# nuggy875/NeRF_pytorch_paeng

Hardware: AMD Instinct MI355X
Metric: rays/sec (4096-ray batch, 64c+128f samples) + 800×800 frame render ms (higher is better)
Workload: dtype f32

## Files before the change

nerf_pytorch_paeng_amd/csrc/layout.h:

```cpp
#pragma once
#include <stdint.h>
#include <stddef.h>

namespace minerf {

constexpr int QUAD_BYTES = 1024;
constexpr int SLOT_QUADS = 16;
constexpr int SLOT_BYTES = QUAD_BYTES * SLOT_QUADS;
constexpr int HEADER_BYTES = 1024;
constexpr uint32_t BLOB_MAGIC = 0x4D494E46u;

__host__ __device__ constexpr int pe_ksteps(int L) { return ((3 * L + 2 + 3) / 4) * 4; }

constexpr int KERNEL_LX = 10, KERNEL_LD = 4;

constexpr int MAX_KERNEL_WIDTH = 512;
__host__ __device__ constexpr int kernel_width(int W) { return W <= 128 ? 128 : (W <= 256 ? 256 : (W <= 384 ? 384 : 512)); }
__host__ __device__ constexpr bool wide_kernel_width(int Wk) { return Wk > 256; }
__host__ __device__ constexpr int pe_ksteps16(int L) { return (((3 * L + 1) / 2 + 1 + 3) / 4) * 4; }
__host__ __device__ constexpr bool native_width(int W) { return W == 128 || W == 256; }

struct BlobLayout {
    uint32_t stream_off;
    uint32_t stream_bytes_hoist;
    uint32_t stream_bytes_full;
    uint32_t side_off;
    uint32_t side_floats;
    uint32_t bias_trunk;
    uint32_t bias_feat;
    uint32_t bias_d;
    uint32_t dens_w;
    uint32_t dens_b;
    uint32_t color_w;
    uint32_t color_b;
    uint32_t wdir_t;
    uint32_t total_bytes;
};

__host__ __device__ inline uint32_t round_up_u32(uint32_t v, uint32_t m) { return (v + m - 1) / m * m; }

inline BlobLayout make_layout(int D, int W_net, int skip, int , int ) {
    constexpr int L_x = KERNEL_LX, L_d = KERNEL_LD;
    const int W = kernel_width(W_net);
    BlobLayout b{};
    const int NT = W / 32;
    const int in_d = 3 + 6 * L_d;
    const uint32_t pe_quads = (uint32_t)(pe_ksteps(L_x) / 4) * NT;
    const uint32_t h_quads = (uint32_t)(W / 2 / 4) * NT;
    uint32_t quads = pe_quads;
    for (int l = 1; l < D; ++l) quads += h_quads + ((skip >= 0 && l == skip + 1) ? pe_quads : 0);
    quads += h_quads;
    quads += (uint32_t)(W / 2 / 4) * (NT / 2);
    b.stream_off = HEADER_BYTES;
    b.stream_bytes_hoist = round_up_u32(quads, SLOT_QUADS) * QUAD_BYTES;
    uint32_t full = round_up_u32(quads, SLOT_QUADS) + round_up_u32((uint32_t)(pe_ksteps(L_d) / 4) * (NT / 2), SLOT_QUADS);
    b.stream_bytes_full = full * QUAD_BYTES;
    b.side_off = b.stream_off + b.stream_bytes_full;
    uint32_t f = 0;
    b.bias_trunk = f; f += (uint32_t)D * W;
    b.bias_feat = f;  f += W;
    b.bias_d = f;     f += W / 2;
    b.dens_w = f;     f += W;
    b.dens_b = f;     f += 4;
    b.color_w = f;    f += 3 * (W / 2);
    b.color_b = f;    f += 4;
    b.wdir_t = f;     f += (uint32_t)in_d * (W / 2);
    b.side_floats = round_up_u32(f, 4);
    b.total_bytes = b.side_off + b.side_floats * 4;
    return b;
}

struct ParamOffsets {
    uint32_t w_x[16], b_x[16];
    int in_l[16];
    uint32_t w_d, b_d, w_feat, b_feat, w_dens, b_dens, w_color, b_color;
    uint32_t total;
};

inline ParamOffsets make_param_offsets(int D, int W, int skip, int L_x, int L_d) {
    ParamOffsets p{};
    const int in_x = 3 + 6 * L_x, in_d = 3 + 6 * L_d;
    uint32_t f = 0;
    for (int l = 0; l < D; ++l) {
        p.in_l[l] = (l == 0) ? in_x : ((skip >= 0 && l == skip + 1) ? W + in_x : W);
        p.w_x[l] = f; f += (uint32_t)W * p.in_l[l];
        p.b_x[l] = f; f += W;
    }
    p.w_d = f;     f += (uint32_t)(W / 2) * (W + in_d);
    p.b_d = f;     f += W / 2;
    p.w_feat = f;  f += (uint32_t)W * W;
    p.b_feat = f;  f += W;
    p.w_dens = f;  f += W;
    p.b_dens = f;  f += 1;
    p.w_color = f; f += 3 * (W / 2);
    p.b_color = f; f += 3;
    p.total = f;
    return p;
}

inline uint32_t bwd_stream_bytes(int D, int W) {
    const uint32_t NT = W / 32;
    const uint32_t quads = (uint32_t)(W / 16) * NT + (uint32_t)D * (uint32_t)(W / 8) * NT;
    return round_up_u32(quads, SLOT_QUADS) * QUAD_BYTES;
}
// ... 3 lines not shown
```

nerf_pytorch_paeng_amd/csrc/mlp_train.hip:

```cpp
#include <type_traits>
#include <vector>
#include "mlp_core.h"

namespace minerf {

int stage_embed(const float*, const float*, int64_t, int, int, int, float*, hipStream_t);
int dgrad_f16s(const mi_nerf_net*, const void*, const float*, const float*, const float*, const unsigned*, const unsigned*, float*, float*, float*, int64_t, int,
               long long, long long, const unsigned*, hipStream_t);

struct DgradArgs {
    const char* stream;
    unsigned stream_bytes;
    const float* side;
    unsigned side_floats, o_dens_w, o_color_w;
    const float* d_raw;
    const unsigned* mask_h;
    const unsigned* mask_g;
    float* delta_h;
    float* delta_f;
    float* delta_d;
    long long P;
    long long n_valid;
    long long n_wtiles;
    int S, tpr;
// ... 66 lines not shown
                    h2[4 * q + e] = mask_apply(v, q, e, mg);
                }
            }
        }
        acc_zero<NT>(acc);
        {
            float* row = a.delta_d + idx * (W / 2) + 4 * hh;
            auto hook = [&](int kq, int t) __attribute__((always_inline)) { if (t == NT - 1) store_chunk(h2, kq, row); };
            gemm_part<NT, HN / 2, NT, AL>(acc, h2, aq, smem, ring, lane, hook);
        }
        acc_to_b<NT, false>(acc, h);
        acc_zero<NT>(acc);
        {
            float* row = a.delta_f + idx * W + 4 * hh;
            auto hook = [&](int kq, int t) __attribute__((always_inline)) { if (t == NT - 1) store_chunk(h, kq, row); };
            gemm_part<NT, HN, NT, AL>(acc, h, aq, smem, ring, lane, hook);
        }
        {
            const unsigned mw[4] = {mhv[0], mhv[1], mhv[2], mhv[3]};
            if (a.D > 1) mhv = *(const u32x4*)(a.mask_h + (((long long)(a.D - 2) * a.n_wtiles + wt) * 64 + lane) * 4);
            const float ds = dr[3];
#pragma unroll
            for (int q = 0; q < 4 * NT; ++q) {
                const f32x4 wv = *(const f32x4*)(dw + 8 * q + 4 * hh);
#pragma unroll
                for (int e = 0; e < 4; ++e)
                    h[4 * q + e] = mask_apply(__builtin_fmaf(wv[e], ds, acc[q >> 2][4 * (q & 3) + e]), q, e, mw);
            }
        }
#pragma unroll 1
        for (int l = a.D - 1; l > 0; --l) {
            float* row = a.delta_h + ((long long)l * a.P + idx) * W + 4 * hh;
            acc_zero<NT>(acc);
            auto hook = [&](int kq, int t) __attribute__((always_inline)) { if (t == NT - 1) store_chunk(h, kq, row); };
            gemm_part<NT, HN, NT, AL>(acc, h, aq, smem, ring, lane, hook);
            const unsigned mw[4] = {mhv[0], mhv[1], mhv[2], mhv[3]};
            if (l > 1) mhv = *(const u32x4*)(a.mask_h + (((long long)(l - 2) * a.n_wtiles + wt) * 64 + lane) * 4);
#pragma unroll
            for (int q = 0; q < 4 * NT; ++q)
#pragma unroll
                for (int e = 0; e < 4; ++e) h[4 * q + e] = mask_apply(acc[q >> 2][4 * (q & 3) + e], q, e, mw);
        }
        store_rows<NT>(h, a.delta_h + idx * W + 4 * hh, valid);
    }
    asm volatile("s_waitcnt vmcnt(0)" ::: "memory");
    __syncthreads();
}

constexpr int WG_MAXB = 12;
struct WgradArgs {
    const float* dlt[WG_MAXB]; const float* x[WG_MAXB];
    int ldd[WG_MAXB], ldx[WG_MAXB], M[WG_MAXB], N[WG_MAXB];
    int want_bias[WG_MAXB];
    long long P;
    float* partial;
    float* bpartial;
    int slices;
};
struct ReduceBatch {
    float* out[WG_MAXB]; float* bias[WG_MAXB];
    int ldo[WG_MAXB], M[WG_MAXB], N[WG_MAXB];
};

typedef unsigned u32x4 __attribute__((ext_vector_type(4)));
__device__ __forceinline__ __amdgpu_buffer_rsrc_t wg_rsrc(const float* base, long long row0, long long ld, long long P, int rows) {
    long long left = P - row0;
    left = left < 0 ? 0 : (left > rows ? rows : left);
    return __builtin_amdgcn_make_buffer_rsrc((void*)(base + row0 * ld), 0, (int)(left * ld * 4), 0x00020000);
}
__global__ __launch_bounds__(256) __attribute__((amdgpu_waves_per_eu(1, 1)))
void wgrad_big_kernel(const WgradArgs a) {
    constexpr int U = 6;
    __shared__ f32x4 bshare[2][64];
    const int lane = threadIdx.x & 63;
    const int wave = __builtin_amdgcn_readfirstlane(threadIdx.x >> 6);
    const int i = lane & 31, kh = lane >> 5;
    const unsigned nwg = gridDim.x * gridDim.y, v = blockIdx.y * gridDim.x + blockIdx.x;
    const unsigned xcd = v & 7, slot = v >> 3;
    const unsigned full = nwg >> 3, rem = nwg & 7;
    const unsigned flat = xcd * full + (xcd < rem ? xcd : rem) + slot;
    const int b = (int)(flat / gridDim.x);
    const unsigned slice = flat - (unsigned)b * gridDim.x;
    const int wm = wave >> 1, wn = wave & 1;
    const int m0 = wm * 128, n0 = wn * 128;
    const bool aok = m0 + 4 * i < a.M[b], bok = n0 + 4 * i < a.N[b];
    const float* abase = a.dlt[b];
    const float* bbase = a.x[b];
    const long long ldd = a.ldd[b], ldx = a.ldx[b];
    const bool want_bias = a.want_bias[b] != 0;

    f32x16 acc[4][4];
#pragma unroll
    for (int tm = 0; tm < 4; ++tm)
#pragma unroll
        for (int tn = 0; tn < 4; ++tn)
#pragma unroll
            for (int r = 0; r < 16; ++r) acc[tm][tn][r] = 0.0f;
    f32x4 bsum = {0.f, 0.f, 0.f, 0.f};

    const long long slices = gridDim.x;
    unsigned voa[U], vob[U];
#pragma unroll
    for (int u = 0; u < U; ++u) {
        voa[u] = aok ? (unsigned)(((2 * u + kh) * ldd + m0 + 4 * i) * 4) : 0x80000000u;
        vob[u] = bok ? (unsigned)(((2 * u + kh) * ldx + n0 + 4 * i) * 4) : 0x80000000u;
    }
    long long req_group = slice;
    f32x4 ca[U], cb[U], na[U], nb[U], fa[U], fb[U];
    __amdgpu_buffer_rsrc_t ra, rb;
    auto open_group = [&]() __attribute__((always_inline)) {
        const long long row0 = req_group * (2 * U);
        ra = wg_rsrc(abase, row0, ldd, a.P, 2 * U);
        rb = wg_rsrc(bbase, row0, ldx, a.P, 2 * U);
        req_group += slices;
    };
    auto request = [&](int u, f32x4& A, f32x4& B) __attribute__((always_inline)) {
        A = __builtin_bit_cast(f32x4, __builtin_amdgcn_raw_buffer_load_b128(ra, voa[u], 0, 0));
        B = __builtin_bit_cast(f32x4, __builtin_amdgcn_raw_buffer_load_b128(rb, vob[u], 0, 0));
    };
    open_group();
#pragma unroll
    for (int u = 0; u < U; ++u) request(u, ca[u], cb[u]);
    open_group();
#pragma unroll
    for (int u = 0; u < U; ++u) request(u, na[u], nb[u]);
    auto step = [&](auto PAR, f32x4 (&A)[U], f32x4 (&B)[U], f32x4 (&FA)[U], f32x4 (&FB)[U]) __attribute__((always_inline)) {
        constexpr int par = decltype(PAR)::value;
        open_group();
#pragma unroll
        for (int u = 0; u < U; ++u) {
#pragma unroll
            for (int tm = 0; tm < 4; ++tm)
#pragma unroll
                for (int tn = 0; tn < 4; ++tn)
                    acc[tm][tn] = __builtin_amdgcn_mfma_f32_32x32x2f32(A[u][tm], B[u][tn], acc[tm][tn], 0, 0, 0);
            if ((u & 1) == par) bsum += A[u];
            request(u, FA[u], FB[u]);
            __builtin_amdgcn_sched_barrier(0);
        }
    };
    const long long all_groups = (a.P + 2 * U - 1) / (2 * U);
    const long long n_groups = (all_groups + slices - 1) / slices;
    auto loop = [&](auto PAR) __attribute__((always_inline)) {
        long long g = 0;
        do {
            step(PAR, ca, cb, fa, fb);
            step(PAR, na, nb, ca, cb);
            step(PAR, fa, fb, na, nb);
            g += 3;
        } while (g < n_groups);
    };
    if (!want_bias) loop(std::integral_constant<int, -1>{});
    else if (wn == 0) loop(std::integral_constant<int, 0>{});
    else loop(std::integral_constant<int, 1>{});
    const int lane_o = (int)__builtin_amdgcn_mbcnt_hi(~0u, __builtin_amdgcn_mbcnt_lo(~0u, 0u));
    const int i_o = lane_o & 31, kh_o = lane_o >> 5;
    float* out = a.partial + ((size_t)b * a.slices + slice) * (256 * 256);
// ... 8 lines not shown
            *(f32x4*)(out + (size_t)m * 256 + n0 + 4 * i_o) = v;
        }
    if (want_bias) {
        if (wn == 1) bshare[wm][lane_o] = bsum;
        __syncthreads();
        if (wn == 0) {
            bsum += bshare[wm][lane_o];
            f32x4 sv;
#pragma unroll
            for (int e = 0; e < 4; ++e) sv[e] = bsum[e] + __shfl_xor(bsum[e], 32, 64);
            if (kh_o == 0) *(f32x4*)(a.bpartial + ((size_t)b * a.slices + slice) * 256 + m0 + 4 * i_o) = sv;
        }
    }
}

typedef _Float16 f16x8 __attribute__((ext_vector_type(8)));
__global__ __launch_bounds__(256) void absmax_kernel(const float* __restrict__ x, long long n, unsigned* __restrict__ out_bits) {
    float m = 0.0f;
    const long long n4 = ((uintptr_t)x & 15) == 0 ? n >> 2 : 0;
    for (long long i = (long long)blockIdx.x * 256 + threadIdx.x; i < n4; i += (long long)gridDim.x * 256) {
        const f32x4 v = ((const f32x4*)x)[i];
        m = __builtin_fmaxf(__builtin_fmaxf(m, __builtin_fmaxf(__builtin_fabsf(v[0]), __builtin_fabsf(v[1]))), __builtin_fmaxf(__builtin_fabsf(v[2]), __builtin_fabsf(v[3])));
    }
    for (long long i = 4 * n4 + (long long)blockIdx.x * 256 + threadIdx.x; i < n; i += (long long)gridDim.x * 256) m = __builtin_fmaxf(m, __builtin_fabsf(x[i]));
#pragma unroll
    for (int o = 32; o > 0; o >>= 1) m = __builtin_fmaxf(m, __shfl_xor(m, o, 64));
    if ((threadIdx.x & 63) == 0 && m == m) atomicMax(out_bits, __float_as_uint(m));
}
static void launch_absmax(const float* x, long long n, unsigned* out_bits, hipStream_t st) {
    long long blocks = (n / 4 + 255) / 256;
    blocks = blocks < 1 ? 1 : (blocks > 4096 ? 4096 : blocks);
    hipLaunchKernelGGL(absmax_kernel, dim3((unsigned)blocks), dim3(256), 0, st, x, n, out_bits);
}
template <bool S>
__device__ __forceinline__ void split_pair(float v0, float v1, float s, unsigned& hi, unsigned& lo) {
    if constexpr (S) { v0 *= s; v1 *= s; }
    asm("v_cvt_pk_f16_f32 %0, %1, %2" : "=v"(hi) : "v"(v0), "v"(v1));
    asm("v_fma_mixlo_f16 %0, %1, -1.0, %2 op_sel_hi:[1,0,0]\n\tv_fma_mixhi_f16 %0, %1, -1.0, %3 op_sel:[1,0,0] op_sel_hi:[1,0,0]"
        : "=&v"(lo) : "v"(hi), "v"(v0), "v"(v1));
}
template <int BIAS>
__device__ __forceinline__ void wgrad_f16s_body(const WgradArgs& a, const unsigned* absmax_bits, f32x4 (*bshare)[64]) {
    const int lane = threadIdx.x & 63;
    const int wave = __builtin_amdgcn_readfirstlane(threadIdx.x >> 6);
    const int i = lane & 31, kh = lane >> 5;
    const unsigned nwg = gridDim.x * gridDim.y, v = blockIdx.y * gridDim.x + blockIdx.x;
    const unsigned xcd = v & 7, slot = v >> 3;
    const unsigned full = nwg >> 3, rem = nwg & 7;
    const unsigned flat = xcd * full + (xcd < rem ? xcd : rem) + slot;
    const int b = (int)(flat / gridDim.x);
    const unsigned slice = flat - (unsigned)b * gridDim.x;
    const int wm = wave >> 1, wn = wave & 1;
    const int m0 = wm * 128, n0 = wn * 128;
    const bool aok = m0 + 4 * i < a.M[b], bok = n0 + 4 * i < a.N[b];
    const float* abase = a.dlt[b];
    const float* bbase = a.x[b];
    const long long ldd = a.ldd[b], ldx = a.ldx[b];
    const unsigned mb = __builtin_amdgcn_readfirstlane((int)*absmax_bits);
    int e = (int)((mb >> 23) & 255u) - 127;
    if (mb == 0u || e < -100) e = -100;
    if (e > 100) e = 100;
    const float sc = __uint_as_float((unsigned)(127 + 7 - e) << 23), inv_sc = __uint_as_float((unsigned)(127 - 7 + e) << 23);

    f32x16 acc[4][4];
#pragma unroll
    for (int tm = 0; tm < 4; ++tm)
#pragma unroll
        for (int tn = 0; tn < 4; ++tn)
#pragma unroll
            for (int r = 0; r < 16; ++r) acc[tm][tn][r] = 0.0f;
    f32x4 bsum = {0.f, 0.f, 0.f, 0.f};

    constexpr int GROUP = 32;
    const long long slices = gridDim.x;
    unsigned voa[4], vob[4];
#pragma unroll
    for (int r = 0; r < 4; ++r) {
        voa[r] = aok ? (unsigned)(((8 * kh + r) * ldd + m0 + 4 * i) * 4) : 0x80000000u;
        vob[r] = bok ? (unsigned)(((8 * kh + r) * ldx + n0 + 4 * i) * 4) : 0x80000000u;
    }
    long long req_group = slice;
    struct Unit { f32x4 A[4], B[4]; };
    auto request = [&](int q, Unit& u) __attribute__((always_inline)) {
        const long long row0 = req_group * GROUP + 16 * (q >> 1) + 4 * (q & 1);
        const __amdgpu_buffer_rsrc_t ra = wg_rsrc(abase, row0, ldd, a.P, 12), rb = wg_rsrc(bbase, row0, ldx, a.P, 12);
#pragma unroll
        for (int r = 0; r < 4; ++r) {
            u.A[r] = __builtin_bit_cast(f32x4, __builtin_amdgcn_raw_buffer_load_b128(ra, voa[r], 0, 0));
            u.B[r] = __builtin_bit_cast(f32x4, __builtin_amdgcn_raw_buffer_load_b128(rb, vob[r], 0, 0));
        }
    };
    auto open_group = [&]() __attribute__((always_inline)) { req_group += slices; };
    unsigned ahi[4][4], alo[4][4], bhi[4][4], blo[4][4];
    auto convert = [&](int h, const Unit& u) __attribute__((always_inline)) {
#pragma unroll
        for (int t = 0; t < 4; ++t)
#pragma unroll
            for (int pr = 0; pr < 2; ++pr) {
                split_pair<true>(u.A[2 * pr][t], u.A[2 * pr + 1][t], sc, ahi[t][2 * h + pr], alo[t][2 * h + pr]);
                split_pair<false>(u.B[2 * pr][t], u.B[2 * pr + 1][t], 1.0f, bhi[t][2 * h + pr], blo[t][2 * h + pr]);
            }
        if constexpr (BIAS) {
#pragma unroll
            for (int r = 0; r < 4; ++r) bsum += u.A[r];
        }
    };
    auto mfmas = [&]() __attribute__((always_inline)) {
        f16x8 AH[4], AL[4], BH[4], BL[4];
#pragma unroll
        for (int t = 0; t < 4; ++t) {
            u32x4 w;
            w[0] = ahi[t][0]; w[1] = ahi[t][1]; w[2] = ahi[t][2]; w[3] = ahi[t][3]; AH[t] = __builtin_bit_cast(f16x8, w);
            w[0] = alo[t][0]; w[1] = alo[t][1]; w[2] = alo[t][2]; w[3] = alo[t][3]; AL[t] = __builtin_bit_cast(f16x8, w);
            w[0] = bhi[t][0]; w[1] = bhi[t][1]; w[2] = bhi[t][2]; w[3] = bhi[t][3]; BH[t] = __builtin_bit_cast(f16x8, w);
            w[0] = blo[t][0]; w[1] = blo[t][1]; w[2] = blo[t][2]; w[3] = blo[t][3]; BL[t] = __builtin_bit_cast(f16x8, w);
        }
#pragma unroll
        for (int tm = 0; tm < 4; ++tm)
#pragma unroll
            for (int tn = 0; tn < 4; ++tn) {
                acc[tm][tn] = __builtin_amdgcn_mfma_f32_32x32x16_f16(AH[tm], BH[tn], acc[tm][tn], 0, 0, 0);
                acc[tm][tn] = __builtin_amdgcn_mfma_f32_32x32x16_f16(AH[tm], BL[tn], acc[tm][tn], 0, 0, 0);
                acc[tm][tn] = __builtin_amdgcn_mfma_f32_32x32x16_f16(AL[tm], BH[tn], acc[tm][tn], 0, 0, 0);
            }
    };
    Unit u0, u1, u2, u3;
    request(0, u0); request(1, u1); request(2, u2); request(3, u3);
    const long long all_groups = (a.P + GROUP - 1) / GROUP;
    const long long n_groups = (all_groups + slices - 1) / slices;
    for (long long g = 0; g < n_groups; ++g) {
        open_group();
// ... 165 lines not shown
#pragma unroll
    for (int q = 0; q < NN; ++q) {
        const float v = nsum[q] + __shfl_xor(nsum[q], 32, 64);
        if (kh == 0) sums[wave * (Wp + Np) + Wp + 32 * q + i] = v;
    }
    __syncthreads();
    for (int c = threadIdx.x; c < Wp + Np; c += 256) {
        const float v = ((sums[c] + sums[(Wp + Np) + c]) + sums[2 * (Wp + Np) + c]) + sums[3 * (Wp + Np) + c];
        if (c < Wp) { if (a.wsum) a.wsum[(size_t)blockIdx.x * Wp + c] = v; }
        else if (a.nsum) a.nsum[(size_t)blockIdx.x * Np + (c - Wp)] = v;
    }
}

__global__ __launch_bounds__(256) void reduce_partial_kernel(const float* __restrict__ partial, const float* __restrict__ bpartial,
                                                              int slices, int Mp, int Np, int M, int N, float* __restrict__ out, int ldo,
                                                              float* __restrict__ bias, int bias_pitch, int transposed) {
    __shared__ float red[4][64];
    const int g = threadIdx.x >> 6, o = threadIdx.x & 63;
    const int idx = blockIdx.x * 64 + o;
    const int total = M * N + (bias ? M : 0);
    float acc = 0.0f;
    if (idx < M * N) {
        const int m = idx / N, n = idx - m * N;
        const float* p = partial + (transposed ? (size_t)n * Np + m : (size_t)m * Np + n);
        const size_t stride = (size_t)Mp * Np;
        float s[8] = {0.f, 0.f, 0.f, 0.f, 0.f, 0.f, 0.f, 0.f};
        int sl = g;
        for (; sl + 28 < slices; sl += 32) {
#pragma unroll
            for (int k = 0; k < 8; ++k) s[k] += p[(size_t)(sl + 4 * k) * stride];
        }
        for (; sl < slices; sl += 4) s[0] += p[(size_t)sl * stride];
        acc = ((s[0] + s[1]) + (s[2] + s[3])) + ((s[4] + s[5]) + (s[6] + s[7]));
    } else if (idx < total) {
        const int m = idx - M * N;
        for (int sl = g; sl < slices; sl += 4) acc += bpartial[(size_t)sl * bias_pitch + m];
    }
    red[g][o] = acc;
    __syncthreads();
    if (g == 0 && idx < total) {
        const float v = ((red[0][o] + red[1][o]) + red[2][o]) + red[3][o];
        if (idx < M * N) { const int m = idx / N, n = idx - m * N; out[(size_t)m * ldo + n] = v; }
        else bias[idx - M * N] = v;
    }
}

__global__ __launch_bounds__(256) void reduce_batch_kernel(const float* __restrict__ partial, const float* __restrict__ bpartial, int slices,
                                                            const ReduceBatch rb) {
    __shared__ float red[4][64];
    const int b = blockIdx.y;
    const int M = rb.M[b], N = rb.N[b];
    const int g = threadIdx.x >> 6, o = threadIdx.x & 63;
    const int idx = blockIdx.x * 64 + o;
    const int total = M * N + (rb.bias[b] ? M : 0);
    float acc = 0.0f;
    if (idx < M * N) {
        const int m = idx / N, n = idx - m * N;
        const float* p = partial + (size_t)b * slices * 65536 + (size_t)m * 256 + n;
        float s[8] = {0.f, 0.f, 0.f, 0.f, 0.f, 0.f, 0.f, 0.f};
        int sl = g;
        for (; sl + 28 < slices; sl += 32) {
#pragma unroll
            for (int k = 0; k < 8; ++k) s[k] += p[(size_t)(sl + 4 * k) * 65536];
        }
        for (; sl < slices; sl += 4) s[0] += p[(size_t)sl * 65536];
        acc = ((s[0] + s[1]) + (s[2] + s[3])) + ((s[4] + s[5]) + (s[6] + s[7]));
    } else if (idx < total) {
        const int m = idx - M * N;
        for (int sl = g; sl < slices; sl += 4) acc += bpartial[((size_t)b * slices + sl) * 256 + m];
    }
    red[g][o] = acc;
    __syncthreads();
    if (g == 0 && idx < total) {
        const float v = ((red[0][o] + red[1][o]) + red[2][o]) + red[3][o];
        if (idx < M * N) { const int m = idx / N, n = idx - m * N; rb.out[b][(size_t)m * rb.ldo[b] + n] = v; }
        else rb.bias[b][idx - M * N] = v;
    }
}

__global__ __launch_bounds__(256) void pack_apply_kernel(const int32_t* __restrict__ map, const float* __restrict__ flat, long long n,
                                                          float* __restrict__ blob) {
    const long long i = (long long)blockIdx.x * 256 + threadIdx.x;
    if (i >= n) return;
    const int32_t m = map[i];
    blob[i] = m > 0 ? flat[m - 1] : 0.0f;
}

static int num_cus_t() { return device_cus(); }

static inline size_t al256(size_t v) { return (v + 255) & ~(size_t)255; }
constexpr size_t WGRAD_OVERRUN_PAD = 128 * 1024;

constexpr size_t WGRAD_PARTIAL_FLOATS = (size_t)256 * 256 * 256 + (size_t)256 * 256;

int train_layout(const mi_nerf_net* net, int64_t n_rays, int S, mi_nerf_train_layout* L) {
    MN_CHECK_ARG(net && L, "NULL net/layout");
    MN_CHECK_ARG(native_width(net->W), "the training kernels exist for W = 128 and 256 (got %d; inference pads narrower networks)", net->W);
    MN_CHECK_ARG(net->D >= 2 && net->D <= 16, "unsupported depth D=%d", net->D);
    MN_CHECK_ARG(n_rays >= 0 && S >= 1, "bad sizes n_rays=%lld S=%d", (long long)n_rays, S);
    const size_t p = (size_t)n_rays * S, W = (size_t)net->W, D = (size_t)net->D;
    const size_t n_wtiles = (size_t)n_rays * ((S + 31) / 32);
    const size_t in_all = (size_t)(3 + 6 * net->L_x) + (size_t)(3 + 6 * net->L_d);
    size_t off = 0;
    L->stash_h = off; off += al256(D * p * W * 4);
    L->stash_f = off; off += al256(p * W * 4);
    L->stash_g = off; off += al256(p * (W / 2) * 4) + WGRAD_OVERRUN_PAD;
    L->mask_h = off;  off += al256(D * n_wtiles * 64 * 16);
    L->mask_g = off;  off += al256(n_wtiles * 64 * 8);
    L->stash_bytes = off;
    off = 0;
    L->delta_h = off; off += al256(D * p * W * 4);
    L->delta_f = off; off += al256(p * W * 4);
    L->delta_d = off; off += al256(p * (W / 2) * 4) + WGRAD_OVERRUN_PAD;
    L->emb = off;     off += al256(p * in_all * 4);
    L->partial = off; off += al256(WGRAD_PARTIAL_FLOATS * 4);
    off += 256;
    L->work_bytes = off;
    return MI_NERF_OK;
}

struct WideProduct { const float* dlt; int ldd, M; const float* x; int ldx, N; float* out; int ldo; float* bias; };

static int run_wgrad_batch(const WideProduct* pr, int n, long long P, float* partial, hipStream_t st, const unsigned* absmax = nullptr) {
    MN_CHECK_ARG(n >= 1 && n <= WG_MAXB, "%d wide products in one batch (at most WG_MAXB)", n);
    WgradArgs a{};
    ReduceBatch rb{};
    int max_total = 0;
    for (int b = 0; b < n; ++b) {
        const WideProduct& q = pr[b];
        MN_CHECK_ARG(q.M <= 256 && q.N <= 256 && q.M % 4 == 0 && q.N % 4 == 0 && q.ldd % 4 == 0 && q.ldx % 4 == 0 &&
                     ((uintptr_t)q.dlt & 15) == 0 && ((uintptr_t)q.x & 15) == 0,
                     "wgrad operands must be at most 256 wide, 16-byte aligned, with pitches of 4 floats");
        a.dlt[b] = q.dlt; a.x[b] = q.x; a.ldd[b] = q.ldd; a.ldx[b] = q.ldx; a.M[b] = q.M; a.N[b] = q.N; a.want_bias[b] = q.bias != nullptr;
        rb.out[b] = q.out; rb.bias[b] = q.bias; rb.ldo[b] = q.ldo; rb.M[b] = q.M; rb.N[b] = q.N;
        const int total = q.M * q.N + (q.bias ? q.M : 0);
        if (total > max_total) max_total = total;
    }
    int slices = num_cus_t() / n;
    const long long all_groups = (P + 11) / 12;
    if (slices > all_groups) slices = (int)all_groups;
    if (slices < 1) slices = 1;
    MN_CHECK_ARG((size_t)n * slices * (65536 + 256) <= WGRAD_PARTIAL_FLOATS, "internal: wgrad partial buffer too small");
    a.P = P; a.slices = slices;
    a.partial = partial;
    a.bpartial = partial + (size_t)n * slices * 65536;
    if (absmax) hipLaunchKernelGGL(wgrad_f16s_kernel, dim3(slices, n), dim3(256), 0, st, a, absmax);
    else hipLaunchKernelGGL(wgrad_big_kernel, dim3(slices, n), dim3(256), 0, st, a);
    MN_LAUNCH_CHECK("wgrad_big_kernel");
    hipLaunchKernelGGL(reduce_batch_kernel, dim3((max_total + 63) / 64, n), dim3(256), 0, st, (const float*)partial, (const float*)a.bpartial,
                       slices, rb);
    MN_LAUNCH_CHECK("reduce_batch_kernel");
    return MI_NERF_OK;
}

static int run_wgrad(const float* dlt, int ldd, int M, const float* x, int ldx, int N, long long P, float* out, int ldo, float* bias,
                     float* partial, hipStream_t st) {
    if (M > 64 && N > 64) {
        const WideProduct q{dlt, ldd, M, x, ldx, N, out, ldo, bias};
        return run_wgrad_batch(&q, 1, P, partial, st);
    }
    const bool delta_is_wide = M >= N;
    NarrowArgs a{};
    a.wide = delta_is_wide ? dlt : x; a.ldw = delta_is_wide ? ldd : ldx; a.Mw = delta_is_wide ? M : N;
    a.nar = delta_is_wide ? x : dlt;  a.ldn = delta_is_wide ? ldx : ldd; a.Nn = delta_is_wide ? N : M;
    a.P = P;
    MN_CHECK_ARG(a.Mw <= 256 && a.Nn <= 64 && a.Mw % 4 == 0 && a.ldw % 4 == 0 && ((uintptr_t)a.wide & 15) == 0,
                 "unsupported narrow wgrad shape %d x %d", M, N);
    const int WQ = a.Mw > 128 ? 2 : 1, NN = a.Nn > 32 ? 2 : 1;
    const int Wp = 128 * WQ, Np = 32 * NN;
    const size_t per_slice = (size_t)Wp * Np + Wp + Np;
    long long wslices = 4LL * num_cus_t();
    long long pps = (P + wslices - 1) / wslices;
    pps = (pps + 23) / 24 * 24;
    wslices = (P + pps - 1) / pps;
    const long long slices = (wslices + 3) / 4;
    MN_CHECK_ARG((size_t)slices * per_slice <= WGRAD_PARTIAL_FLOATS, "internal: wgrad partial buffer too small");
    a.pps = (int)pps;
    a.partial = partial;
    float* wsum = partial + (size_t)slices * Wp * Np;
    float* nsum = wsum + (size_t)slices * Wp;
    a.wsum = (bias && delta_is_wide) ? wsum : nullptr;
    a.nsum = (bias && !delta_is_wide) ? nsum : nullptr;
    const dim3 grid((unsigned)slices);
    const bool bw = a.wsum != nullptr, bn = a.nsum != nullptr;
#define MN_NARROW(WQ_, NN_)                                                                                                   \
    do {                                                                                                                      \
        if (bw) hipLaunchKernelGGL((wgrad_narrow_kernel<WQ_, NN_, true, false>), grid, dim3(256), 0, st, a);                  \
        else if (bn) hipLaunchKernelGGL((wgrad_narrow_kernel<WQ_, NN_, false, true>), grid, dim3(256), 0, st, a);             \
// ... 39 lines not shown
        }
        MN_LAUNCH_CHECK("absmax_kernel");
    }
    if (n_wide)
        if (int rc = run_wgrad_batch(pr, n_wide, P, (float*)scratch, st, absmax)) return rc;
    for (int b = 0; b < n; ++b)
        if (!(M[b] > 64 && N[b] > 64))
            if (int rc = run_wgrad(dlt[b], ldd[b], M[b], x[b], ldx[b], N[b], P, out[b], ldo[b], bias ? bias[b] : nullptr, (float*)scratch, st)) return rc;
    return MI_NERF_OK;
}

template <int W>
static int launch_dgrad(const DgradArgs& a, hipStream_t st) {
    const size_t lds = RING_BYTES + (size_t)a.side_floats * 4;
    MN_CHECK_ARG(lds <= 160 * 1024, "LDS budget exceeded: %zu bytes", lds);
    auto kern = mlp_dgrad_kernel<W>;
    static LdsOptIn opt_in = {};
    if (int rc = ensure_lds_opt_in(opt_in, (const void*)kern)) return rc;
    const long long n_wg = (a.n_wtiles + 3) / 4;
    const int grid = (int)(n_wg < (long long)num_cus_t() ? n_wg : (long long)num_cus_t());
    hipLaunchKernelGGL(kern, dim3(grid), dim3(256), lds, st, a);
    MN_LAUNCH_CHECK("mlp_dgrad_kernel");
    return MI_NERF_OK;
}

int mlp_backward_fp32(const mi_nerf_net* net, const void* packed_fwd, const void* packed_bwd, const float* rays, const float* z,
                      int64_t n_rays, int S, const float* d_raw, const void* stash, void* work, size_t work_bytes, float* grads,
                      int stage, hipStream_t st, const float* x_dev, int64_t n_rows, int mode) {
    MN_CHECK_ARG(net != nullptr, "net is NULL");
    MN_CHECK_ARG(net->L_x >= 0 && net->L_x <= KERNEL_LX && net->L_d >= 0 && net->L_d <= KERNEL_LD, "unsupported encoding L_x=%d L_d=%d", net->L_x, net->L_d);
    MN_CHECK_ARG(net->skip >= -1, "bad skip=%d", net->skip);
    MN_CHECK_ARG(n_rays >= 0 && S >= 1, "bad sizes n_rays=%lld S=%d", (long long)n_rays, S);
    const long long Ppad = (long long)n_rays * S;
    const long long P = x_dev ? n_rows : Ppad;
    MN_CHECK_ARG(!x_dev || (S == 32 && n_rows >= 0 && n_rays == (n_rows + 31) / 32), "embedded mode wants (n_rays, S) = (ceil(n / 32), 32)");
    mi_nerf_train_layout L;
    if (int rc = train_layout(net, n_rays, S, &L)) return rc;
    if (P == 0) {
        if (grads && stage != 1) {
            MN_CHECK_ARG(net->D >= 1 && net->D <= 16 && (net->W == 128 || net->W == 256), "unsupported network D=%d W=%d", net->D, net->W);
            MN_HIP(hipMemsetAsync(grads, 0, (size_t)make_param_offsets(net->D, net->W, net->skip, net->L_x, net->L_d).total * 4, st));
        }
        if ((mode & 3) && work && work_bytes >= L.work_bytes)
            MN_HIP(hipMemsetAsync((char*)work + L.partial + al256(WGRAD_PARTIAL_FLOATS * 4), 0, 8, st));
        return MI_NERF_OK;
    }
    MN_CHECK_ARG(packed_fwd && packed_bwd && (x_dev || (rays && z)) && d_raw && stash && work && grads, "NULL device pointer");
    MN_CHECK_ARG(work_bytes >= L.work_bytes, "workspace too small: %zu < %zu", work_bytes, L.work_bytes);
    const int D = net->D, W = net->W;
    const int in_x = 3 + 6 * net->L_x, in_d = 3 + 6 * net->L_d, in_all = in_x + in_d;
    const BlobLayout BL = make_layout(D, W, net->skip, net->L_x, net->L_d);
    const ParamOffsets po = make_param_offsets(D, W, net->skip, net->L_x, net->L_d);
    const float* stash_h = (const float*)((const char*)stash + L.stash_h);
    const float* stash_f = (const float*)((const char*)stash + L.stash_f);
    const float* stash_g = (const float*)((const char*)stash + L.stash_g);
    float* delta_h = (float*)((char*)work + L.delta_h);
    float* delta_f = (float*)((char*)work + L.delta_f);
    float* delta_d = (float*)((char*)work + L.delta_d);
    float* emb = (float*)((char*)work + L.emb);
    float* partial = (float*)((char*)work + L.partial);

    DgradArgs a{};
    a.stream = (const char*)packed_bwd + HEADER_BYTES;
    a.stream_bytes = bwd_stream_bytes(D, W);
    a.side = (const float*)((const char*)packed_fwd + BL.side_off);
    a.side_floats = BL.side_floats; a.o_dens_w = BL.dens_w; a.o_color_w = BL.color_w;
    a.d_raw = d_raw;
    a.mask_h = (const unsigned*)((const char*)stash + L.mask_h);
    a.mask_g = (const unsigned*)((const char*)stash + L.mask_g);
    a.delta_h = delta_h; a.delta_f = delta_f; a.delta_d = delta_d;
    a.S = S; a.tpr = (S + 31) / 32;
    a.P = Ppad; a.n_valid = P; a.n_wtiles = (long long)n_rays * a.tpr; a.D = D;
    unsigned* absmax = nullptr;
    if (mode & 3) {
        MN_CHECK_ARG(W == 256 && !x_dev, "the split-precision backward is built for W=256 and the ray entry point");
        absmax = (unsigned*)((char*)work + L.partial + al256(WGRAD_PARTIAL_FLOATS * 4));
        MN_HIP(hipMemsetAsync(absmax, 0, 8, st));
        launch_absmax(d_raw, (long long)P * 4, absmax, st);
        MN_LAUNCH_CHECK("absmax_kernel");
    }
    if (mode & 2) {
        if (int rc = dgrad_f16s(net, packed_bwd, a.side + a.o_color_w, a.side + a.o_dens_w, d_raw, a.mask_h, a.mask_g, delta_h, delta_f, delta_d, n_rays, S,
                                Ppad, P, absmax, st)) return rc;
    } else {
        if (int rc = (W == 256 ? launch_dgrad<256>(a, st) : launch_dgrad<128>(a, st))) return rc;
    }
    if (stage == 1) return MI_NERF_OK;

    const float* embc = x_dev;
    if (!x_dev) {
        if (int rc = stage_embed(rays, z, n_rays, S, net->L_x, net->L_d, emb, st)) return rc;
        embc = emb;
    }
    const size_t PW = (size_t)Ppad * W;
    if (!(mode & 1)) absmax = nullptr;
    const float* h_last = stash_h + (size_t)(D - 1) * PW;
    {
        WideProduct pr[WG_MAXB];
        int n = 0;
        auto flush = [&]() -> int {
            const int rc = n ? run_wgrad_batch(pr, n, P, partial, st, absmax) : MI_NERF_OK;
            n = 0;
            return rc;
        };
        for (int l = 1; l < D; ++l) {
            const bool cat = po.in_l[l] != W;
            pr[n++] = WideProduct{delta_h + (size_t)l * PW, W, W, stash_h + (size_t)(l - 1) * PW, W, W, grads + po.w_x[l] + (cat ? in_x : 0),
                                  po.in_l[l], grads + po.b_x[l]};
            if (n == WG_MAXB) if (int rc = flush()) return rc;
        }
        pr[n++] = WideProduct{delta_f, W, W, h_last, W, W, grads + po.w_feat, W, grads + po.b_feat};
        if (n == WG_MAXB) if (int rc = flush()) return rc;
        pr[n++] = WideProduct{delta_d, W / 2, W / 2, stash_f, W, W, grads + po.w_d, W + in_d, grads + po.b_d};
        if (int rc = flush()) return rc;
    }
    if (int rc = run_wgrad(delta_h, W, W, embc, in_all, in_x, P, grads + po.w_x[0], in_x, grads + po.b_x[0], partial, st)) return rc;
    for (int l = 1; l < D; ++l)
        if (po.in_l[l] != W)
            if (int rc = run_wgrad(delta_h + (size_t)l * PW, W, W, embc, in_all, in_x, P, grads + po.w_x[l], po.in_l[l], nullptr, partial, st)) return rc;
    if (int rc = run_wgrad(d_raw + 3, 4, 1, h_last, W, W, P, grads + po.w_dens, W, grads + po.b_dens, partial, st)) return rc;
    if (int rc = run_wgrad(delta_d, W / 2, W / 2, embc + in_x, in_all, in_d, P, grads + po.w_d + W, W + in_d, nullptr, partial, st)) return rc;
    if (int rc = run_wgrad(d_raw, 4, 3, stash_g, W / 2, W / 2, P, grads + po.w_color, W / 2, grads + po.b_color, partial, st)) return rc;
    return MI_NERF_OK;
}

int pack_apply(const int32_t* map_dev, const float* flat_dev, size_t blob_bytes, void* blob_dev, hipStream_t st) {
    MN_CHECK_ARG(map_dev && flat_dev && blob_dev, "NULL device pointer");
    MN_CHECK_ARG(blob_bytes % 4 == 0, "blob size must be a multiple of 4");
    const long long n = (long long)(blob_bytes / 4);
    if (n == 0) return MI_NERF_OK;
    hipLaunchKernelGGL(pack_apply_kernel, dim3((unsigned)((n + 255) / 256)), dim3(256), 0, st, map_dev, flat_dev, n, (float*)blob_dev);
    MN_LAUNCH_CHECK("pack_apply_kernel");
    return MI_NERF_OK;
}

}
```

nerf_pytorch_paeng_amd/csrc/pack.cpp:

```cpp
#include <hip/hip_runtime.h>
#include <string.h>
#include "half_layout.h"

namespace minerf {

namespace {

struct KStep { int lo, hi; };

std::vector<KStep> enc_ksteps(int LK, int L, int base) {
    std::vector<KStep> ks;
    for (int s = 0; s < 3 * LK; ++s) {
        const int k = s / 3, c = s % 3;
        if (k < L) ks.push_back({base + 3 + 6 * k + c, base + 3 + 6 * k + 3 + c});
        else ks.push_back({-1, -1});
    }
    ks.push_back({base + 0, base + 1});
    ks.push_back({base + 2, -1});
    while ((int)ks.size() < pe_ksteps(LK)) ks.push_back({-1, -1});
    return ks;
}

std::vector<KStep> act_ksteps(int W, int base, int n_real = -1) {
    if (n_real < 0) n_real = W;
// ... 68 lines not shown
}


void emit_part_t(std::vector<float>& stream, const float* Wm, int n_rows, int ld, int col_base, int n_feat, int NT,
                 const std::vector<KStep>& ks) {
    const int KQ = (int)ks.size() / 4;
    for (int kq = 0; kq < KQ; ++kq)
        for (int T = 0; T < NT; ++T)
            for (int lane = 0; lane < 64; ++lane)
                for (int j = 0; j < 4; ++j) {
                    const KStep& k = ks[4 * kq + j];
                    const int row = (lane >> 5) ? k.hi : k.lo;
                    const int n = 32 * T + (lane & 31);
                    stream.push_back((row >= 0 && row < n_rows && n < n_feat) ? Wm[(size_t)row * ld + col_base + n] : 0.0f);
                }
    const size_t slot_floats = SLOT_BYTES / 4;
    while (stream.size() % slot_floats) stream.push_back(0.0f);
}

}

int pack_fp32(const mi_nerf_net* net, const mi_nerf_params* p, void* blob, size_t blob_bytes) {
    MN_CHECK_ARG(net->W >= 2 && net->W <= MAX_KERNEL_WIDTH, "unsupported width W=%d (the fp32 inference kernels run 2 <= W <= %d)", net->W, MAX_KERNEL_WIDTH);
    const int D = net->D, Wn = net->W, Hn = Wn / 2, W = kernel_width(Wn), NT = W / 32;
    const int in_x = 3 + 6 * net->L_x, in_d = 3 + 6 * net->L_d;
    const BlobLayout L = make_layout(D, Wn, net->skip, net->L_x, net->L_d);
    MN_CHECK_ARG(blob_bytes >= L.total_bytes, "blob too small: %zu < %u", blob_bytes, L.total_bytes);
    memset(blob, 0, L.total_bytes);

    std::vector<float> stream;
    stream.reserve(L.stream_bytes_full / 4);
    const bool w16 = wide_kernel_width(W);
    if (w16) {
        const int NT16 = W / 16;
        emit_part16(stream, p->linear_x_w[0], Wn, in_x, NT16, enc_ksteps16(KERNEL_LX, net->L_x, 0));
        for (int l = 1; l < D; ++l) {
            const bool cat = (net->skip >= 0 && l == net->skip + 1);
            const int n_in = cat ? Wn + in_x : Wn;
            if (cat) emit_part16(stream, p->linear_x_w[l], Wn, n_in, NT16, enc_ksteps16(KERNEL_LX, net->L_x, 0));
            emit_part16(stream, p->linear_x_w[l], Wn, n_in, NT16, act_ksteps16(W, cat ? in_x : 0, Wn));
        }
        emit_part16(stream, p->linear_feat_w, Wn, Wn, NT16, act_ksteps16(W, 0, Wn));
        emit_part16(stream, p->linear_d_w, Hn, Wn + in_d, NT16 / 2, act_ksteps16(W, 0, Wn));
        MN_CHECK_ARG(stream.size() * 4 == L.stream_bytes_hoist, "internal: hoisted stream %zu != %u", stream.size() * 4, L.stream_bytes_hoist);
        emit_part16(stream, p->linear_d_w, Hn, Wn + in_d, NT16 / 2, enc_ksteps16(KERNEL_LD, net->L_d, Wn));
    } else {
    emit_part(stream, p->linear_x_w[0], Wn, in_x, NT, enc_ksteps(KERNEL_LX, net->L_x, 0));
    for (int l = 1; l < D; ++l) {
        const bool cat = (net->skip >= 0 && l == net->skip + 1);
        const int n_in = cat ? Wn + in_x : Wn;
        if (cat) emit_part(stream, p->linear_x_w[l], Wn, n_in, NT, enc_ksteps(KERNEL_LX, net->L_x, 0));
        emit_part(stream, p->linear_x_w[l], Wn, n_in, NT, act_ksteps(W, cat ? in_x : 0, Wn));
    }
    emit_part(stream, p->linear_feat_w, Wn, Wn, NT, act_ksteps(W, 0, Wn));
    emit_part(stream, p->linear_d_w, Hn, Wn + in_d, NT / 2, act_ksteps(W, 0, Wn));
    MN_CHECK_ARG(stream.size() * 4 == L.stream_bytes_hoist, "internal: hoisted stream %zu != %u", stream.size() * 4, L.stream_bytes_hoist);
    emit_part(stream, p->linear_d_w, Hn, Wn + in_d, NT / 2, enc_ksteps(KERNEL_LD, net->L_d, Wn));
    }
    MN_CHECK_ARG(stream.size() * 4 == L.stream_bytes_full, "internal: full stream %zu != %u", stream.size() * 4, L.stream_bytes_full);

    uint32_t* hdr = (uint32_t*)blob;
    hdr[0] = BLOB_MAGIC; hdr[1] = w16 ? 6 : 1; hdr[2] = D; hdr[3] = W; hdr[4] = (uint32_t)net->skip; hdr[5] = KERNEL_LX; hdr[6] = KERNEL_LD;
    hdr[13] = net->L_x; hdr[14] = net->L_d; hdr[15] = Wn;
    hdr[7] = L.stream_off; hdr[8] = L.stream_bytes_hoist; hdr[9] = L.stream_bytes_full; hdr[10] = L.side_off; hdr[11] = L.side_floats;
    hdr[12] = 4;
    memcpy((char*)blob + L.stream_off, stream.data(), L.stream_bytes_full);

    float* side = (float*)((char*)blob + L.side_off);
    for (int l = 0; l < D; ++l) memcpy(side + L.bias_trunk + (size_t)l * W, p->linear_x_b[l], Wn * 4);
    memcpy(side + L.bias_feat, p->linear_feat_b, Wn * 4);
    memcpy(side + L.bias_d, p->linear_d_b, Hn * 4);
    memcpy(side + L.dens_w, p->linear_density_w, Wn * 4);
    side[L.dens_b] = p->linear_density_b[0];
    for (int c = 0; c < 3; ++c) memcpy(side + L.color_w + (size_t)c * (W / 2), p->linear_color_w + (size_t)c * Hn, Hn * 4);
    memcpy(side + L.color_b, p->linear_color_b, 3 * 4);
    for (int f = 0; f < in_d; ++f)
        for (int n = 0; n < Hn; ++n) side[L.wdir_t + (size_t)f * (W / 2) + n] = p->linear_d_w[(size_t)n * (Wn + in_d) + Wn + f];
    return MI_NERF_OK;
}

size_t packed_bytes_bwd(const mi_nerf_net* net) {
    if (!native_width(net->W)) {
        set_error("the training kernels exist for W = 128 and 256 (got %d; inference pads narrower networks)", net->W);
        return 0;
    }
    return HEADER_BYTES + (size_t)bwd_stream_bytes(net->D, net->W);
}

int pack_bwd_fp32(const mi_nerf_net* net, const mi_nerf_params* p, void* blob, size_t blob_bytes) {
    MN_CHECK_ARG(native_width(net->W), "the training kernels exist for W = 128 and 256 (got %d; inference pads narrower networks)", net->W);
    const int D = net->D, W = net->W, NT = W / 32;
    const int in_x = 3 + 6 * net->L_x, in_d = 3 + 6 * net->L_d;
    const size_t total = packed_bytes_bwd(net);
    MN_CHECK_ARG(blob_bytes >= total, "blob too small: %zu < %zu", blob_bytes, total);
    memset(blob, 0, total);
    std::vector<float> stream;
    stream.reserve((total - HEADER_BYTES) / 4);
    emit_part_t(stream, p->linear_d_w, W / 2, W + in_d, 0, W, NT, act_ksteps(W / 2, 0));
    emit_part_t(stream, p->linear_feat_w, W, W, 0, W, NT, act_ksteps(W, 0));
    for (int l = D - 1; l >= 1; --l) {
        const bool cat = (net->skip >= 0 && l == net->skip + 1);
        emit_part_t(stream, p->linear_x_w[l], W, cat ? W + in_x : W, cat ? in_x : 0, W, NT, act_ksteps(W, 0));
    }
    MN_CHECK_ARG(stream.size() * 4 + HEADER_BYTES == total, "internal: backward stream %zu != %zu", stream.size() * 4, total - HEADER_BYTES);
    uint32_t* hdr = (uint32_t*)blob;
    hdr[0] = BLOB_MAGIC; hdr[1] = 2; hdr[2] = D; hdr[3] = W; hdr[4] = (uint32_t)net->skip; hdr[5] = net->L_x; hdr[6] = net->L_d;
    hdr[7] = HEADER_BYTES; hdr[8] = (uint32_t)(total - HEADER_BYTES);
    memcpy((char*)blob + HEADER_BYTES, stream.data(), stream.size() * 4);
    return MI_NERF_OK;
// ... 37 lines not shown
```

Measured before the change: 489,800.

## Compute feature-layer weight grads algebraically from a small G matrix instead of wide products

The backward pass no longer runs the wide weight-gradient products for linear_feat and linear_d (feature part) over all points. It computes one product G = delta_d^T · h_last, plus the density weight gradient folded into the same launch as a second operand row. A small finish kernel then derives dW_feat, db_feat and dW_d from G, the bias sums and the packed forward weights. This removes a P-length reduction and the stash_f read. The cost is extra argument plumbing and a layout-dependent index into the packed stream, which is checked at pack time.

```diff
diff --git a/nerf_pytorch_paeng_amd/csrc/layout.h b/nerf_pytorch_paeng_amd/csrc/layout.h
--- a/nerf_pytorch_paeng_amd/csrc/layout.h
+++ b/nerf_pytorch_paeng_amd/csrc/layout.h
@@ -35,7 +35,12 @@
     uint32_t color_b;
     uint32_t wdir_t;
     uint32_t total_bytes;
+    uint32_t feat_part, d_part;
 };
+
+__host__ __device__ constexpr uint32_t act_part_index(int NT_out, int n, int f) {
+    return (uint32_t)((((f >> 3) * NT_out + (n >> 5)) * 64 + (n & 31) + 32 * ((f >> 2) & 1)) * 4 + (f & 3));
+}
 
 __host__ __device__ inline uint32_t round_up_u32(uint32_t v, uint32_t m) { return (v + m - 1) / m * m; }
 
@@ -49,7 +54,9 @@
     const uint32_t h_quads = (uint32_t)(W / 2 / 4) * NT;
     uint32_t quads = pe_quads;
     for (int l = 1; l < D; ++l) quads += h_quads + ((skip >= 0 && l == skip + 1) ? pe_quads : 0);
+    b.feat_part = quads * (QUAD_BYTES / 4);
     quads += h_quads;
+    b.d_part = quads * (QUAD_BYTES / 4);
     quads += (uint32_t)(W / 2 / 4) * (NT / 2);
     b.stream_off = HEADER_BYTES;
     b.stream_bytes_hoist = round_up_u32(quads, SLOT_QUADS) * QUAD_BYTES;
diff --git a/nerf_pytorch_paeng_amd/csrc/mlp_train.hip b/nerf_pytorch_paeng_amd/csrc/mlp_train.hip
--- a/nerf_pytorch_paeng_amd/csrc/mlp_train.hip
+++ b/nerf_pytorch_paeng_amd/csrc/mlp_train.hip
@@ -142,6 +142,7 @@
     const float* dlt[WG_MAXB]; const float* x[WG_MAXB];
     int ldd[WG_MAXB], ldx[WG_MAXB], M[WG_MAXB], N[WG_MAXB];
     int want_bias[WG_MAXB];
+    const float* dlt2[WG_MAXB]; int ldd2[WG_MAXB], M2[WG_MAXB];
     long long P;
     float* partial;
     float* bpartial;
@@ -150,6 +151,7 @@
 struct ReduceBatch {
     float* out[WG_MAXB]; float* bias[WG_MAXB];
     int ldo[WG_MAXB], M[WG_MAXB], N[WG_MAXB];
+    float* out2[WG_MAXB]; float* bias2[WG_MAXB]; int row2[WG_MAXB];
 };
 
 typedef unsigned u32x4 __attribute__((ext_vector_type(4)));
@@ -173,10 +175,12 @@
     const unsigned slice = flat - (unsigned)b * gridDim.x;
     const int wm = wave >> 1, wn = wave & 1;
     const int m0 = wm * 128, n0 = wn * 128;
-    const bool aok = m0 + 4 * i < a.M[b], bok = n0 + 4 * i < a.N[b];
-    const float* abase = a.dlt[b];
+    const bool up = wm == 1 && a.dlt2[b] != nullptr;
+    const float* abase = up ? a.dlt2[b] : a.dlt[b];
     const float* bbase = a.x[b];
-    const long long ldd = a.ldd[b], ldx = a.ldx[b];
+    const long long ldd = up ? a.ldd2[b] : a.ldd[b], ldx = a.ldx[b];
+    const int ac0 = up ? 0 : m0;
+    const bool aok = ac0 + 4 * i < (up ? a.M2[b] : a.M[b]), bok = n0 + 4 * i < a.N[b];
     const bool want_bias = a.want_bias[b] != 0;
 
     f32x16 acc[4][4];
@@ -192,7 +196,7 @@
     unsigned voa[U], vob[U];
 #pragma unroll
     for (int u = 0; u < U; ++u) {
-        voa[u] = aok ? (unsigned)(((2 * u + kh) * ldd + m0 + 4 * i) * 4) : 0x80000000u;
+        voa[u] = aok ? (unsigned)(((2 * u + kh) * ldd + ac0 + 4 * i) * 4) : 0x80000000u;
         vob[u] = bok ? (unsigned)(((2 * u + kh) * ldx + n0 + 4 * i) * 4) : 0x80000000u;
     }
     long long req_group = slice;
@@ -307,10 +311,12 @@
     const unsigned slice = flat - (unsigned)b * gridDim.x;
     const int wm = wave >> 1, wn = wave & 1;
     const int m0 = wm * 128, n0 = wn * 128;
-    const bool aok = m0 + 4 * i < a.M[b], bok = n0 + 4 * i < a.N[b];
-    const float* abase = a.dlt[b];
+    const bool up = wm == 1 && a.dlt2[b] != nullptr;
+    const float* abase = up ? a.dlt2[b] : a.dlt[b];
     const float* bbase = a.x[b];
-    const long long ldd = a.ldd[b], ldx = a.ldx[b];
+    const long long ldd = up ? a.ldd2[b] : a.ldd[b], ldx = a.ldx[b];
+    const int ac0 = up ? 0 : m0;
+    const bool aok = ac0 + 4 * i < (up ? a.M2[b] : a.M[b]), bok = n0 + 4 * i < a.N[b];
     const unsigned mb = __builtin_amdgcn_readfirstlane((int)*absmax_bits);
     int e = (int)((mb >> 23) & 255u) - 127;
     if (mb == 0u || e < -100) e = -100;
@@ -331,7 +337,7 @@
     unsigned voa[4], vob[4];
 #pragma unroll
     for (int r = 0; r < 4; ++r) {
-        voa[r] = aok ? (unsigned)(((8 * kh + r) * ldd + m0 + 4 * i) * 4) : 0x80000000u;
+        voa[r] = aok ? (unsigned)(((8 * kh + r) * ldd + ac0 + 4 * i) * 4) : 0x80000000u;
         vob[r] = bok ? (unsigned)(((8 * kh + r) * ldx + n0 + 4 * i) * 4) : 0x80000000u;
     }
     long long req_group = slice;
@@ -603,10 +609,21 @@
     const int M = rb.M[b], N = rb.N[b];
     const int g = threadIdx.x >> 6, o = threadIdx.x & 63;
     const int idx = blockIdx.x * 64 + o;
-    const int total = M * N + (rb.bias[b] ? M : 0);
+    const int nb = rb.bias[b] ? M : 0, n2 = rb.out2[b] ? N + 1 : 0;
+    const int total = M * N + nb + n2;
+    int m = 0, n = 0;
+    bool is_bias = false;
+    float* dst = nullptr;
+    if (idx < M * N) { m = idx / N; n = idx - m * N; dst = rb.out[b] + (size_t)m * rb.ldo[b] + n; }
+    else if (idx < M * N + nb) { is_bias = true; m = idx - M * N; dst = rb.bias[b] + m; }
+    else if (idx < total) {
+        const int e = idx - M * N - nb;
+        m = rb.row2[b];
+        if (e < N) { n = e; dst = rb.out2[b] + n; }
+        else { is_bias = true; dst = rb.bias2[b]; }
+    }
     float acc = 0.0f;
-    if (idx < M * N) {
-        const int m = idx / N, n = idx - m * N;
+    if (dst && !is_bias) {
         const float* p = partial + (size_t)b * slices * 65536 + (size_t)m * 256 + n;
         float s[8] = {0.f, 0.f, 0.f, 0.f, 0.f, 0.f, 0.f, 0.f};
         int sl = g;
@@ -616,16 +633,56 @@
         }
         for (; sl < slices; sl += 4) s[0] += p[(size_t)sl * 65536];
         acc = ((s[0] + s[1]) + (s[2] + s[3])) + ((s[4] + s[5]) + (s[6] + s[7]));
-    } else if (idx < total) {
-        const int m = idx - M * N;
+    } else if (dst) {
         for (int sl = g; sl < slices; sl += 4) acc += bpartial[((size_t)b * slices + sl) * 256 + m];
     }
     red[g][o] = acc;
     __syncthreads();
-    if (g == 0 && idx < total) {
-        const float v = ((red[0][o] + red[1][o]) + red[2][o]) + red[3][o];
-        if (idx < M * N) { const int m = idx / N, n = idx - m * N; rb.out[b][(size_t)m * rb.ldo[b] + n] = v; }
-        else rb.bias[b][idx - M * N] = v;
+    if (g == 0 && dst) *dst = ((red[0][o] + red[1][o]) + red[2][o]) + red[3][o];
+}
+
+struct FinishArgs {
+    const float* G;
+    const float* s;
+    const float* wfeat; const float* wd;
+    const float* bfeat;
+    float* dw_feat; float* db_feat; float* dw_d;
+    int ld_wd;
+};
+template <int W>
+__global__ __launch_bounds__(256) void feature_finish_kernel(const FinishArgs a) {
+    constexpr int H = W / 2, NT = W / 32;
+    constexpr int NA = W * W / 256, NC = H * W / 256;
+    const int blk = blockIdx.x, tid = threadIdx.x;
+    float acc[4] = {0.f, 0.f, 0.f, 0.f};
+    if (blk < NA) {
+        const int idx = blk * 256 + tid, j = idx / W, k = idx - j * W;
+        const float* w = a.wd + act_part_index(NT / 2, 0, j);
+        const float* g = a.G + k;
+        for (int m = 0; m < H; m += 4)
+#pragma unroll
+            for (int e = 0; e < 4; ++e) acc[e] = __builtin_fmaf(w[((m + e) >> 5) * 256 + ((m + e) & 31) * 4], g[(size_t)(m + e) * W], acc[e]);
+        a.dw_feat[idx] = (acc[0] + acc[1]) + (acc[2] + acc[3]);
+    } else if (blk < NA + NC) {
+        const int idx = (blk - NA) * 256 + tid, m = idx / W, j = idx - m * W;
+        const f32x4* w = (const f32x4*)a.wfeat + (j >> 5) * 64 + (j & 31);
+        const float* g = a.G + (size_t)m * W;
+        for (int kq = 0; kq < W / 8; ++kq)
+#pragma unroll
+            for (int hh = 0; hh < 2; ++hh) {
+                const f32x4 wv = w[kq * NT * 64 + 32 * hh];
+#pragma unroll
+                for (int e = 0; e < 4; ++e) acc[e] = __builtin_fmaf(g[8 * kq + 4 * hh + e], wv[e], acc[e]);
+            }
+        a.dw_d[(size_t)m * a.ld_wd + j] = __builtin_fmaf(a.s[m], a.bfeat[j], (acc[0] + acc[1]) + (acc[2] + acc[3]));
+    } else {
+        const int j = (blk - NA - NC) * 256 + tid;
+        if (j >= W) return;
+        const float* w = a.wd + act_part_index(NT / 2, 0, j);
+        for (int m = 0; m < H; m += 4)
+#pragma unroll
+            for (int e = 0; e < 4; ++e) acc[e] = __builtin_fmaf(w[((m + e) >> 5) * 256 + ((m + e) & 31) * 4], a.s[m + e], acc[e]);
+        a.db_feat[j] = (acc[0] + acc[1]) + (acc[2] + acc[3]);
     }
 }
 
@@ -670,7 +727,10 @@
     return MI_NERF_OK;
 }
 
-struct WideProduct { const float* dlt; int ldd, M; const float* x; int ldx, N; float* out; int ldo; float* bias; };
+struct WideProduct {
+    const float* dlt; int ldd, M; const float* x; int ldx, N; float* out; int ldo; float* bias;
+    const float* dlt2 = nullptr; int ldd2 = 0, M2 = 0; float* out2 = nullptr; float* bias2 = nullptr; int row2 = 0;
+};
 
 static int run_wgrad_batch(const WideProduct* pr, int n, long long P, float* partial, hipStream_t st, const unsigned* absmax = nullptr) {
     MN_CHECK_ARG(n >= 1 && n <= WG_MAXB, "%d wide products in one batch (at most WG_MAXB)", n);
@@ -684,7 +744,14 @@
                      "wgrad operands must be at most 256 wide, 16-byte aligned, with pitches of 4 floats");
         a.dlt[b] = q.dlt; a.x[b] = q.x; a.ldd[b] = q.ldd; a.ldx[b] = q.ldx; a.M[b] = q.M; a.N[b] = q.N; a.want_bias[b] = q.bias != nullptr;
         rb.out[b] = q.out; rb.bias[b] = q.bias; rb.ldo[b] = q.ldo; rb.M[b] = q.M; rb.N[b] = q.N;
-        const int total = q.M * q.N + (q.bias ? q.M : 0);
+        if (q.dlt2) {
+            MN_CHECK_ARG(q.M <= 128 && q.M2 >= 1 && q.M2 <= 128 && q.ldd2 % 4 == 0 && ((uintptr_t)q.dlt2 & 15) == 0 && q.bias && q.out2 && q.bias2 &&
+                         q.row2 >= 128 && q.row2 < 128 + q.M2,
+                         "a second gradient operand needs M <= 128, a 16-byte aligned operand with a pitch of 4 floats, and a row of its own to keep");
+            a.dlt2[b] = q.dlt2; a.ldd2[b] = q.ldd2; a.M2[b] = q.M2;
+            rb.out2[b] = q.out2; rb.bias2[b] = q.bias2; rb.row2[b] = q.row2;
+        }
+        const int total = q.M * q.N + (q.bias ? q.M : 0) + (q.dlt2 ? q.N + 1 : 0);
         if (total > max_total) max_total = total;
     }
     int slices = num_cus_t() / n;
@@ -830,7 +897,6 @@
     const BlobLayout BL = make_layout(D, W, net->skip, net->L_x, net->L_d);
     const ParamOffsets po = make_param_offsets(D, W, net->skip, net->L_x, net->L_d);
     const float* stash_h = (const float*)((const char*)stash + L.stash_h);
-    const float* stash_f = (const float*)((const char*)stash + L.stash_f);
     const float* stash_g = (const float*)((const char*)stash + L.stash_g);
     float* delta_h = (float*)((char*)work + L.delta_h);
     float* delta_f = (float*)((char*)work + L.delta_f);
@@ -873,6 +939,8 @@
     const size_t PW = (size_t)Ppad * W;
     if (!(mode & 1)) absmax = nullptr;
     const float* h_last = stash_h + (size_t)(D - 1) * PW;
+    float* feat_G = (float*)((char*)work + L.delta_d + al256((size_t)Ppad * (W / 2) * 4));
+    static_assert((size_t)128 * 256 * 4 <= WGRAD_OVERRUN_PAD, "G of a 256-wide network must fit the slack behind delta_d");
     {
         WideProduct pr[WG_MAXB];
         int n = 0;
@@ -887,16 +955,22 @@
                                   po.in_l[l], grads + po.b_x[l]};
             if (n == WG_MAXB) if (int rc = flush()) return rc;
         }
-        pr[n++] = WideProduct{delta_f, W, W, h_last, W, W, grads + po.w_feat, W, grads + po.b_feat};
-        if (n == WG_MAXB) if (int rc = flush()) return rc;
-        pr[n++] = WideProduct{delta_d, W / 2, W / 2, stash_f, W, W, grads + po.w_d, W + in_d, grads + po.b_d};
+        pr[n++] = WideProduct{delta_d, W / 2, W / 2, h_last, W, W, feat_G, W, grads + po.b_d, d_raw, 4, 4, grads + po.w_dens, grads + po.b_dens, 128 + 3};
         if (int rc = flush()) return rc;
+        FinishArgs f{};
+        const float* fstream = (const float*)((const char*)packed_fwd + BL.stream_off);
+        f.G = feat_G; f.s = grads + po.b_d;
+        f.wfeat = fstream + BL.feat_part; f.wd = fstream + BL.d_part; f.bfeat = a.side + BL.bias_feat;
+        f.dw_feat = grads + po.w_feat; f.db_feat = grads + po.b_feat; f.dw_d = grads + po.w_d; f.ld_wd = W + in_d;
+        const int blocks = (W * W + (W / 2) * W) / 256 + 1;
+        if (W == 256) hipLaunchKernelGGL(feature_finish_kernel<256>, dim3(blocks), dim3(256), 0, st, f);
+        else hipLaunchKernelGGL(feature_finish_kernel<128>, dim3(blocks), dim3(256), 0, st, f);
+        MN_LAUNCH_CHECK("feature_finish_kernel");
     }
     if (int rc = run_wgrad(delta_h, W, W, embc, in_all, in_x, P, grads + po.w_x[0], in_x, grads + po.b_x[0], partial, st)) return rc;
     for (int l = 1; l < D; ++l)
         if (po.in_l[l] != W)
             if (int rc = run_wgrad(delta_h + (size_t)l * PW, W, W, embc, in_all, in_x, P, grads + po.w_x[l], po.in_l[l], nullptr, partial, st)) return rc;
-    if (int rc = run_wgrad(d_raw + 3, 4, 1, h_last, W, W, P, grads + po.w_dens, W, grads + po.b_dens, partial, st)) return rc;
     if (int rc = run_wgrad(delta_d, W / 2, W / 2, embc + in_x, in_all, in_d, P, grads + po.w_d + W, W + in_d, nullptr, partial, st)) return rc;
     if (int rc = run_wgrad(d_raw, 4, 3, stash_g, W / 2, W / 2, P, grads + po.w_color, W / 2, grads + po.b_color, partial, st)) return rc;
     return MI_NERF_OK;
diff --git a/nerf_pytorch_paeng_amd/csrc/pack.cpp b/nerf_pytorch_paeng_amd/csrc/pack.cpp
--- a/nerf_pytorch_paeng_amd/csrc/pack.cpp
+++ b/nerf_pytorch_paeng_amd/csrc/pack.cpp
@@ -144,9 +144,19 @@
         if (cat) emit_part(stream, p->linear_x_w[l], Wn, n_in, NT, enc_ksteps(KERNEL_LX, net->L_x, 0));
         emit_part(stream, p->linear_x_w[l], Wn, n_in, NT, act_ksteps(W, cat ? in_x : 0, Wn));
     }
+    MN_CHECK_ARG(stream.size() == L.feat_part, "internal: linear_feat part at %zu != %u", stream.size(), L.feat_part);
     emit_part(stream, p->linear_feat_w, Wn, Wn, NT, act_ksteps(W, 0, Wn));
+    MN_CHECK_ARG(stream.size() == L.d_part, "internal: linear_d part at %zu != %u", stream.size(), L.d_part);
     emit_part(stream, p->linear_d_w, Hn, Wn + in_d, NT / 2, act_ksteps(W, 0, Wn));
     MN_CHECK_ARG(stream.size() * 4 == L.stream_bytes_hoist, "internal: hoisted stream %zu != %u", stream.size() * 4, L.stream_bytes_hoist);
+    for (int f = 0; f < Wn; ++f) {
+        for (int n = 0; n < Wn; ++n)
+            MN_CHECK_ARG(memcmp(&stream[L.feat_part + act_part_index(NT, n, f)], &p->linear_feat_w[(size_t)n * Wn + f], 4) == 0,
+                         "internal: act_part_index misses linear_feat[%d][%d]", n, f);
+        for (int n = 0; n < Hn; ++n)
+            MN_CHECK_ARG(memcmp(&stream[L.d_part + act_part_index(NT / 2, n, f)], &p->linear_d_w[(size_t)n * (Wn + in_d) + f], 4) == 0,
+                         "internal: act_part_index misses linear_d[%d][%d]", n, f);
+    }
     emit_part(stream, p->linear_d_w, Hn, Wn + in_d, NT / 2, enc_ksteps(KERNEL_LD, net->L_d, Wn));
     }
     MN_CHECK_ARG(stream.size() * 4 == L.stream_bytes_full, "internal: full stream %zu != %u", stream.size() * 4, L.stream_bytes_full);
```

New measurement: 489,700. Within noise of the previous version (-0.0%).
